# JuliaQuantumControl/QuantumPropagators.jl

Measured on AMD Instinct MI355X. Metric: Cheby prop_step!/s at N=2^20 CSR fp64 (2^20-row blocks advanced per second), higher is better.
Workload: dtype c128 (complex fp64); 1 GPU; BASELINE configs[1]: Cheby prop_step!, N=2^20 CSR sparse Hermitian H, 16 nnz/row, c128, int32 indices; N_total=1048576, rows_per_gpu=1048576, pattern=banded, n_coeffs=32, device_format=hrb (Hermitian-packed row blocks), parallelism=single GPU

## Files before the change

### quantumpropagators.jl_amd/csrc/device.h

```cpp
#pragma once

#include <hip/hip_runtime.h>

#include "layout_constants.h"

namespace qp {

#define QP_HIP(expr)                                                                         \
  do {                                                                                       \
    hipError_t e__ = (expr);                                                                 \
    if (e__ != hipSuccess) {                                                                 \
      (void)hipGetLastError();  \
      return qp::fail(QP_E_HIP, "%s failed: %s (%s:%d)", #expr, hipGetErrorString(e__), __FILE__, \
                      __LINE__);                                                             \
    }                                                                                        \
  } while (0)

constexpr int kRedBlocks = 256;
constexpr int kThreads = 256;

struct Stats;
struct Tuning;

struct DevMatrix {
  int format = QP_FMT_RBCSR;
  const Tuning* tun = nullptr;
  int64_t nrows = 0, ncols = 0, nnz = 0, stored = 0;
  int64_t nblocks = 0;
  int64_t* bptr = nullptr;
  int32_t* cols = nullptr;
  int64_t* cmeta = nullptr;
  int64_t colbytes = 0;
  double2* vals = nullptr;
  const double* vals_r = nullptr;
  int64_t* rowptr = nullptr;
  int lanes_per_row = 16;
  int64_t* lptr = nullptr;
  int32_t* lcols = nullptr;
  int64_t* lcmeta = nullptr;
  int64_t lcolbytes = 0;
  int32_t* lpos = nullptr;
  int64_t lstored = 0;
  const struct WalkPlan* walk = nullptr;
  const struct ColBlockPlan* cb = nullptr;
  const struct CodedVals* cv = nullptr;
  void* matfree = nullptr;
  int (*matfree_apply)(hipStream_t s, void* self, const double2* x, double2* y, double2 alpha, double2 beta,
                       Stats* st) = nullptr;
  double2* (*matfree_scratch)(void* self) = nullptr;
  int (*matfree_cheby)(hipStream_t s, void* self, const double2* x, const struct ChebyEpi& e, Stats* st) = nullptr;
};

constexpr int kWalkMaxNear = 8;
constexpr int kWalkHalo = 16;
struct WalkPlan {
  int valid = 0;
  int nn = 0, K = 0, z0 = 0;
  int S = 0;
  int xl = 0;
  int64_t glong = 0;
  int64_t glong1 = 0;
  int fd = 0;
  int64_t g = 0;
  int near[kWalkMaxNear] = {0};
  int64_t R0 = 0, R1 = 0, W0 = 0;
  int64_t U0 = 0;
  int ustride = 0;
  int32_t* edge_map = nullptr;
  int64_t n_edge = 0;
};

struct ColBlockPlan {
  int valid = 0;
  int log2w = 17;
  int P = 0;
  int rpt = 2;
  int max_seg = 0;
  int64_t ntiles = 0, nnz = 0;
  int32_t* segptr = nullptr;
  uint16_t* rowoff = nullptr;
  uint32_t* cols = nullptr;
  int64_t* map = nullptr;
  double2* vals = nullptr;
  double* vals_r = nullptr;
  int use_real = 0;
};
struct CodedVals {
// ... 6 lines not shown
  double* tab_r = nullptr;
  int use_real = 0;
};
constexpr int kCbMaxTilesPerWave = 8;
constexpr int kCbMaxSeg = 1024;

struct ChebyEpi {
  const double2* xloc;
  const double2* v0;
  double2* vout;
  const double2* acc_in;
  double2* acc_out;
  double2 c;
  double beta, a_prev, a;
  double2 phase;
  int apply_phase;
  double* check_partials;
  const int32_t* mirror = nullptr;
  double2* slab = nullptr;
  int acc_skip = 0;
  int n_defer = 0;
  double a_d1 = 0.0;
  double a_d2 = 0.0;
};

struct SyncArgs {
  unsigned* signal = nullptr;
  const unsigned* wait = nullptr;
  unsigned wait_target = 0;
  unsigned wait_from_wg = 0;
  unsigned* timeout_flag = nullptr;
  unsigned spin_limit = 1u << 28;
};

struct RowSet {
  const int32_t* block_map = nullptr;
  int64_t nmap = 0;
  bool count = true;
  SyncArgs sync;
  const struct WalkPlan* walk = nullptr;
  int reserve_cu = 0;
};

struct PlainEpi {
  double2* y;
  double2 alpha, beta;
  int beta_zero;
  const double2* norm_part = nullptr;
  const double2* xloc = nullptr;
  double2* qn_out = nullptr;
  double2* hess_slot = nullptr;
  double* norm_slot = nullptr;
  double dt = 1.0, norm_min = 0.0;
  unsigned* flag = nullptr;
  unsigned flag_value = 0;
};

struct Stats {
  uint64_t n_matvec = 0, n_cheby_steps = 0, n_newton_steps = 0, n_restarts = 0, n_launch = 0, n_graph_launch = 0;
  double spmv_bytes = 0;
};

int launch_spmv_cheby(hipStream_t s, const DevMatrix& A, const double2* x, const ChebyEpi& e, Stats* st,
                      const RowSet* rs = nullptr);
int launch_spmv_plain(hipStream_t s, const DevMatrix& A, const double2* x, const PlainEpi& e, Stats* st);
int launch_arnoldi_matvec_dots(hipStream_t s, const DevMatrix& A, const double2* x, const PlainEpi& e, const double2* Q,
                               int64_t ldq, int j, double2* partials, bool* launched, Stats* st);
bool arnoldi_onepass_fits(const DevMatrix& A, int m, int nvec);
int op_part_slots(int nvec);
int launch_arnoldi_onepass_sweep(hipStream_t s, const DevMatrix& A, const double2* start, double s0, double2* Q, int64_t ldq,
                                 double2* const a_buf[2], int m, int nvec, double2* const part[2], double2* gram, double2* hhat,
                                 double* svals, double* nu_dev, double dt, double2* hess_map, double* norms_map, double* nu_map,
                                 unsigned* flags_map, unsigned flag_value, Stats* st);
inline bool walk_shape_supported(int nn, int K, int z0, int xl = 0, int fd = 0) {
  if (fd) return fd == 1 && (xl == 0 || xl == 1) && K == 1 && nn >= 1 && nn <= 2 && (z0 == 0 || z0 == 1);
  if (xl) return (xl == 1 || xl == 2) && nn >= 1 && nn <= 2 && (K == 1 || K == 2) && (z0 == 0 || z0 == 1);
  return nn >= 1 && nn <= 4 && K >= 1 && K <= 4 && (z0 == 0 || z0 == 1);
}
inline bool walk2_shape_supported(int nn, int K, int z0) {
  return (z0 == 0 || z0 == 1) && nn >= 1 && nn <= 4 && K >= 1 && K <= 4;
}
int launch_hrb_walk2_cheby(hipStream_t s, const DevMatrix& A, const WalkPlan& P2, const double2* x, const ChebyEpi& e1,
                           const ChebyEpi& e2, const Tuning& tun, bool* launched);
int launch_hrb_walk_cheby(hipStream_t s, const DevMatrix& A, const double2* x, const ChebyEpi& e, const Tuning& tun,
                          bool* launched, const RowSet* rs = nullptr);
int launch_dense_gemv_cheby(hipStream_t s, const DevMatrix& A, const double2* x, const ChebyEpi& e, Stats* st);
int launch_dense_gemv_plain(hipStream_t s, const DevMatrix& A, const double2* x, const PlainEpi& e, Stats* st);
int launch_dense_zgemm_cheby(hipStream_t s, const DevMatrix& A, const double2* X, int batch, const ChebyEpi& e, Stats* st);
int launch_rbcsr_coded_cheby(hipStream_t s, const DevMatrix& A, const double2* x, const ChebyEpi& e, int64_t nblk,
                             const int32_t* bmap, const SyncArgs& sy, bool wide);
int launch_rbcsr_coded_plain(hipStream_t s, const DevMatrix& A, const double2* x, const PlainEpi& e, int64_t nblk,
                             const int32_t* bmap, const SyncArgs& sy);
int launch_colblock_cheby(hipStream_t s, const DevMatrix& A, const double2* x, const ChebyEpi& e, const Tuning& tun, bool* launched);
int launch_colblock_plain(hipStream_t s, const DevMatrix& A, const double2* x, const PlainEpi& e, const Tuning& tun, bool* launched);
int launch_colblock_gather(hipStream_t s, const ColBlockPlan& P, const double2* src, Stats* st);
int spmv_grid_size(const DevMatrix& A);
inline int dense_gemv_rows_per_wave(int64_t nrows) { return nrows >= 16384 ? 4 : 1; }
inline int dense_gemv_grid(int64_t nrows) {
  const int64_t per_wg = (int64_t)(kThreads / 64) * dense_gemv_rows_per_wave(nrows);
  return (int)((nrows + per_wg - 1) / per_wg);
}
constexpr int kDenseMinDensityPct = 75;
constexpr int kCbWavesPerCu = 16;
constexpr int kCbMinLog2N = 20;
constexpr int kWalkReserveCu = 8;
constexpr int kWalkEdgeSteps = 4;

struct Tuning {
  int rbcsr_variant = 15;
  int arnoldi_mode = 1;
  int arnoldi_onepass = 1;
  int sparse_controls = 1;
  int lattice_fill = 1;
  int arnoldi_fuse_dots = 1;
  int split_spin_log2 = 28;
  int split_dbg = 0;
  int split_mode = 2;
  int liouville_tile32_min_n = 260;
  int liouville_tile32_n = 2048;
  int liouville_fused_n = 320;
  int real_vals = 1;
  int block_map = 1;
  int stencil = 1;
  int acc_defer = 1;
  int cheby_graph = 0;
  int roctx = 0;
  int dense_auto = 1;
  int dense_panel_mfma = 1;
  int colblock = 1;
  int cb_log2w = 0;
  int small_nnz = 8192;
  int newton_pipeline = 1;
  int spmm_rows = 1;
  int spmm_rw = -1;
  int spmm_strip = 0;
  int hrb_walk = 1;
  int walk_waves = 0;
  int walk_pair = -1;
  int value_dict = 1;
  int walk_nt = -1;
  int walk_dbg = 0;
  int walk_min_blocks = 3072;
  int spmm_nt = 1;
};
int device_cu_count();
int* tuning_field(Tuning& t, const char* key);

constexpr int kCoefBlock = 32;
struct CoefBlock {
  double2 c[kCoefBlock];
};

int launch_real_part(hipStream_t s, double* out, const double2* v, int64_t n, Stats* st);
int launch_combine_planes(hipStream_t s, double2* vals, const double2* const* planes_dev, const double2* coefs,
                          int nplanes, int64_t n, double* vals_r, Stats* st);
int launch_sparse_planes_update(hipStream_t s, double2* vals, const double2* base, const int32_t* support, int64_t n_support,
                                const double2* support_vals, int nplanes, const double2* coefs, double* vals_r, Stats* st);


int launch_spmm_cheby(hipStream_t s, const int64_t* rowptr, const int32_t* cols, const double2* vals,
                      const double2* X, int64_t nrows, int64_t nnz, int b, const ChebyEpi& e, const Tuning& tun,
                      bool rows_kernel, const int32_t* order, Stats* st);
constexpr int kSpmmTileMaxEntries = 24;
constexpr int kSpmmTileSlots = 80;
struct SpmmTileShape {
  int nd = 0, K = 0, NN = 0;
  int dfar[kSpmmTileMaxEntries] = {0};
  int dnear[kSpmmTileMaxEntries] = {0};
};
constexpr int kSpmmTileTab = kSpmmTileSlots + 16 * kSpmmTileMaxEntries + 32;
struct SpmmTiles {
  bool built = false;
  int valid = 0;
  int knob = 0;
  SpmmTileShape shape;
  int64_t g = 0, sw = 0;
  int32_t* tiles = nullptr;
  int64_t ntiles = 0;
  int32_t* rest = nullptr;
  int64_t nrest = 0;
  int32_t* tab = nullptr;
  int T = 0;
};
int launch_spmm_tile_cheby(hipStream_t s, const int64_t* rowptr, const int32_t* cols, const double2* vals, const double2* X,
                           int64_t nrows, int64_t nnz, int b, const ChebyEpi& e, const Tuning& tun, const SpmmTiles& P, Stats* st);
inline bool spmm_uses_rows_kernel(const Tuning& tun, int b) { return tun.spmm_rows != 0 && b > 32; }
struct SmallObs {
  const int64_t* rowptr;
// ... 100 lines not shown
```

### quantumpropagators.jl_amd/csrc/engine_cheby.hip

```cpp
#include "engine.h"

void acc_schedule(const double* a, int n_coeffs, bool defer, qp_acc_defer* out) {
  const int nterms = n_coeffs - 1;
  std::vector<char> upd((size_t)nterms + 1, defer ? 0 : 1);
  if (defer) {
    int m0 = nterms;
    for (; m0 >= 1; m0 -= 3) upd[m0] = 1;
    if (m0 + 3 == 3) upd[1] = 1;
  }
  int last_upd = 0;
  for (int m = 1; m <= nterms; ++m) {
    qp_acc_defer& d = out[m - 1];
    d = qp_acc_defer{0, 0, 0.0, 0.0};
    if (upd[m]) {
      d.n_defer = m - last_upd - 1;
      d.a_d1 = (d.n_defer >= 1) ? a[m - 1] : 0.0;
      d.a_d2 = (d.n_defer == 2) ? a[m - 2] : 0.0;
      last_upd = m;
    } else {
      d.skip = 1;
    }
  }
}

// ... 13 lines not shown
}

extern "C" {

int qp_cheby_create(qp_ctx* ctx, int64_t n, qp_cheby** out) {
  QP_TRY
  if (!ctx || !out || n < 0) return qp::fail(QP_E_BAD_ARG, "qp_cheby_create: bad arguments");
  QP_CHECK(use(ctx));
  auto w = std::make_unique<qp_cheby>();
  w->ctx = ctx;
  w->n = n;
  QP_CHECK(dev_alloc(&w->bufA, (size_t)n));
  QP_CHECK(dev_alloc(&w->acc, (size_t)n));
  *out = w.release();
  return QP_OK;
  QP_CATCH
}

int qp_cheby_destroy(qp_cheby* w) {
  QP_TRY
  if (!w) return QP_OK;
  (void)hipSetDevice(w->ctx->device);
  (void)hipStreamSynchronize(w->ctx->stream);
  if (w->bufA) (void)hipFree(w->bufA);
  if (w->bufC) (void)hipFree(w->bufC);
  if (w->bufD) (void)hipFree(w->bufD);
  if (w->acc) (void)hipFree(w->acc);
  if (w->chk_part) (void)hipFree(w->chk_part);
  if (w->chk_out) (void)hipFree(w->chk_out);
  if (w->gexec) (void)hipGraphExecDestroy(w->gexec);
  delete w;
  return QP_OK;
  QP_CATCH
}

int qp_acc_schedule_host(const double* a, int n_coeffs, qp_acc_defer* out) {
  if (!a || !out || n_coeffs < 2) return qp::fail(QP_E_BAD_ARG, "qp_acc_schedule_host: bad arguments");
  acc_schedule(a, n_coeffs, true, out);
  return QP_OK;
}

int qp_cheby_term(qp_operator* op, const qp_state* x, int64_t xoff, const qp_state* v0, qp_state* vout,
                  const qp_state* acc_in, qp_state* acc_out, qp_c128 c, double beta, double a_prev, double a,
                  qp_c128 phase, const qp_acc_defer* defer) {
  QP_TRY
  const bool skip = defer && defer->skip;
  if (!op || !x || (!acc_out && !skip)) return qp::fail(QP_E_BAD_ARG, "qp_cheby_term: NULL argument");
  if (defer && !skip && (defer->n_defer < 0 || defer->n_defer > 2 || (defer->n_defer > 0 && !v0 && (defer->n_defer == 2 || !acc_in))))
    return qp::fail(QP_E_BAD_ARG, "qp_cheby_term: deferred accumulation needs v0");
  const int64_t nr = op->A.nrows;
  if (x->n != op->A.ncols || xoff < 0 || xoff + nr > x->n) return qp::fail(QP_E_BAD_ARG, "qp_cheby_term: x shape / offset mismatch");
  if ((v0 && v0->n != nr) || (vout && vout->n != nr) || (acc_in && acc_in->n != nr) || (acc_out && acc_out->n != nr))
    return qp::fail(QP_E_BAD_ARG, "qp_cheby_term: local vector length mismatch");
  auto overlaps = [&](const qp_state* s) { return s && s->d < x->d + x->n && x->d < s->d + s->n; };
  if (overlaps(vout) || overlaps(acc_out)) return qp::fail(QP_E_BAD_ARG, "qp_cheby_term: outputs must not overlap the gathered x");
  QP_CHECK(use(op->ctx));
  qp::ChebyEpi e;
  e.xloc = x->d + xoff;
  e.v0 = v0 ? v0->d : nullptr;
  e.vout = vout ? vout->d : nullptr;
  e.acc_in = (acc_in && !skip) ? acc_in->d : nullptr;
  e.acc_out = (acc_out && !skip) ? acc_out->d : nullptr;
  e.c = d2(c);
  e.beta = beta;
  e.a_prev = a_prev;
  e.a = a;
  e.phase = d2(phase);
  e.apply_phase = !(phase.re == 1.0 && phase.im == 0.0);
  e.check_partials = nullptr;
  set_defer(e, defer);
  return qp::launch_spmv_cheby(op->ctx->stream, op->A, x->d, e, &op->ctx->stats);
  QP_CATCH
}

static bool walk2_wanted(const qp_operator* op) {
  const qp::Tuning& tun = op->ctx->tun;
  const qp::WalkPlan& Q = op->walk2;
  const DevMatrix& A = op->A;
  if (!Q.valid || tun.walk_pair == 0 || !tun.hrb_walk || (tun.rbcsr_variant & 31) != 15 || A.walk != &op->walk || !op->walk.valid) return false;
  if (op->walk.R1 - op->walk.W0 < tun.walk_min_blocks) return false;
  if (tun.walk_pair == 1) return true;
  const double footprint = (double)(Q.z0 + Q.nn + Q.K) * kRB * (double)A.nblocks * (A.vals_r ? 8.0 : 16.0) + 64.0 * (double)A.nrows;
  if (footprint <= 230e6) return false;
  const int W = kRB - 2 * Q.near[Q.nn - 1];
  const int64_t S2 = (Q.g + W - 1) / W, Jz = ((Q.R1 - Q.W0) * (int64_t)kRB + Q.g - 1) / Q.g;
  const int64_t waves = tun.walk_waves > 0 ? tun.walk_waves : 4 * (int64_t)qp::device_cu_count();
  return Jz / std::max<int64_t>(1, waves / S2) >= 24;
}

int qp_operator_walk2_info(const qp_operator* op, int64_t out[8]) {
  QP_TRY
  if (!op || !out) return qp::fail(QP_E_BAD_ARG, "qp_operator_walk2_info: NULL argument");
  const bool on = walk2_wanted(op);
  const int W = on ? kRB - 2 * op->walk2.near[op->walk2.nn - 1] : 0;
  out[0] = on ? 1 : 0;
  out[1] = on ? op->walk2.W0 : 0;
  out[2] = on ? op->walk2.R1 : 0;
  out[3] = on ? op->walk2.n_edge : 0;
  out[4] = W;
  out[5] = on ? (op->walk2.g + W - 1) / W : 0;
  out[6] = out[7] = 0;
  if (on) {
    const qp::Tuning& tun = op->ctx->tun;
    const int64_t Jz = ((op->walk2.R1 - op->walk2.W0) * (int64_t)kRB + op->walk2.g - 1) / op->walk2.g;
    const int64_t waves = tun.walk_waves > 0 ? tun.walk_waves : 4 * (int64_t)qp::device_cu_count();
    const int64_t L = (Jz + std::max<int64_t>(1, waves / out[5]) - 1) / std::max<int64_t>(1, waves / out[5]);
    out[6] = L;
    out[7] = (Jz + L - 1) / L;
  }
  return QP_OK;
  QP_CATCH
}

static int cheby_step_launches(qp_cheby* w, qp_operator* op, qp_state* psi, const double* a, int n_coeffs, double beta,
                               cplx c, cplx phase, bool check_normalization) {
  qp_ctx* ctx = op->ctx;
  const DevMatrix& A = op->A;
  const int nterms = n_coeffs - 1;
  const int nwg = qp::spmv_grid_size(A);
  double2* P = psi->d;
  double2* B = w->bufA;
  double2* ACC = w->acc;
  double2* result = nullptr;
  std::vector<qp_acc_defer> sched((size_t)nterms);
  acc_schedule(a, n_coeffs, ctx->tun.acc_defer != 0, sched.data());
  bool pairs = !check_normalization && nterms >= 3 && w->bufC && w->bufD && walk2_wanted(op);
  double2 *cur = P, *prev = nullptr;
  double2* spare[2] = {w->bufC, w->bufD};
  bool updated = false;
  auto fill = [&](qp::ChebyEpi& e, int m, const double2* x) {
    e.a_prev = updated ? 0.0 : a[0];
    set_defer(e, &sched[m - 1]);
    if (sched[m - 1].skip) {
      e.acc_in = nullptr;
      e.acc_out = nullptr;
    } else {
      updated = true;
    }
    e.xloc = x;
    e.c = d2(c);
    e.beta = beta;
    e.a = a[m];
    e.phase = d2(phase);
    e.apply_phase = (m == nterms) ? 1 : 0;
  };
  for (int m = 1; m <= nterms; ++m) {
    const bool last = (m == nterms);
    qp::ChebyEpi e;
    if (m == 1) {
      e.v0 = nullptr;
      e.vout = last ? nullptr : B;
      e.acc_in = nullptr;
      e.acc_out = ACC;
      result = ACC;
    } else if (pairs && m + 1 <= nterms && !(sched[m - 1].skip == 0 && sched[m].skip == 0)) {
      const bool last2 = (m + 1 == nterms);
      const bool updated_before = updated;
      qp::ChebyEpi e1, e2;
      e1.v0 = prev;
      e1.vout = spare[0];
      e1.acc_in = updated ? ACC : nullptr;
      e1.acc_out = ACC;
      e1.check_partials = nullptr;
      fill(e1, m, cur);
      e2.v0 = cur;
      e2.vout = last2 ? nullptr : spare[1];
      e2.acc_in = updated ? ACC : nullptr;
      e2.acc_out = ACC;
      e2.check_partials = nullptr;
      fill(e2, m + 1, spare[0]);
      bool launched = false;
      {
        const qp::ScopedRange mv_range(ctx->tun.roctx != 0 || qp::ranges_enabled_by_env(), "matrix-vector product");
        QP_CHECK(qp::launch_hrb_walk2_cheby(ctx->stream, A, op->walk2, cur, e1, e2, ctx->tun, &launched));
        if (launched) {
          qp::RowSet rs;
          rs.block_map = op->walk2.edge_map;
          rs.nmap = op->walk2.n_edge;
          rs.count = false;
          QP_CHECK(qp::launch_spmv_cheby(ctx->stream, A, spare[0], e2, &ctx->stats, &rs));
          ctx->stats.n_launch++;
          ctx->stats.n_matvec += 2;
          ctx->stats.spmv_bytes += 2.0 * (20.0 * (double)A.nnz + 4.0 * (double)(A.nrows + 1) + 80.0 * (double)A.nrows);
        }
      }
      if (launched) {
        result = ACC;
        double2* const y = spare[0];
        double2* const z = spare[1];
        spare[0] = cur;
        spare[1] = prev;
        prev = y;
        cur = z;
        ++m;
        continue;
      }
      updated = updated_before;
      pairs = false;
    }
    if (m > 1) {
      e.v0 = prev;
      e.vout = last ? nullptr : prev;
      e.acc_in = updated ? ACC : nullptr;
      e.acc_out = (last && cur != P && !pairs) ? P : ACC;
      result = e.acc_out;
    }
    fill(e, m, cur);
    e.check_partials = (check_normalization && m >= 2) ? w->chk_part : nullptr;
    {
      const qp::ScopedRange mv_range(ctx->tun.roctx != 0 || qp::ranges_enabled_by_env(), "matrix-vector product");
      QP_CHECK(qp::launch_spmv_cheby(ctx->stream, A, cur, e, &ctx->stats));
    }
    if (e.check_partials)
      QP_CHECK(qp::launch_reduce_triples(ctx->stream, w->chk_part, nwg, w->chk_out + 3 * (m - 1), &ctx->stats));
    if (m == 1) {
      c *= 2.0;
      prev = P;
      cur = B;
    } else {
      std::swap(cur, prev);
    }
  }
  if (result != P)
    QP_HIP(hipMemcpyAsync(P, result, (size_t)psi->n * sizeof(double2), hipMemcpyDeviceToDevice, ctx->stream));
  return QP_OK;
}

int qp_cheby_step(qp_cheby* w, qp_operator* op, qp_state* psi, const double* a, int n_coeffs, double Delta,
                  double E_min, double dt, double wrk_dt, double limit, int check_normalization) {
  QP_TRY
  if (!w || !op || !psi || !a) return qp::fail(QP_E_BAD_ARG, "qp_cheby_step: NULL argument");
  if (op->A.nrows != op->A.ncols || psi->n != op->A.nrows || w->n != psi->n)
    return qp::fail(QP_E_BAD_ARG, "qp_cheby_step: shape mismatch");
  {
    const double x = std::fabs(dt), y = std::fabs(wrk_dt);
    if (!(std::fabs(x - y) <= 1.4901161193847656e-08 * std::max(x, y)))
      return qp::fail(QP_E_DT_MISMATCH, "wrk was initialized for dt=%g, not dt=abs(%g)", wrk_dt, dt);
  }
  if (n_coeffs < 2) return qp::fail(QP_E_TOO_FEW_COEFFS, "Need at least 2 Chebychev coefficients");
  if (!(Delta > 0)) return qp::fail(QP_E_BAD_ARG, "Delta must be positive");
  qp_ctx* ctx = op->ctx;
  QP_CHECK(use(ctx));
  const qp::ScopedRange step_range(ctx->tun.roctx != 0 || qp::ranges_enabled_by_env(), "prop_step!");
  const double beta = (Delta / 2) + E_min;
  cplx c = (dt > 0) ? cplx(0, -2.0) / Delta : cplx(0, 2.0) / Delta;
  const cplx phase = std::exp(cplx(0, -1) * beta * dt);
  const int nterms = n_coeffs - 1;
  const DevMatrix& A = op->A;
  const int nwg = qp::spmv_grid_size(A);
  if (check_normalization) {
    if (w->chk_wg < nwg) {
      if (w->chk_part) QP_HIP(hipFree(w->chk_part));
      QP_CHECK(dev_alloc(&w->chk_part, (size_t)3 * nwg));
      w->chk_wg = nwg;
    }
    if (w->chk_terms < nterms) {
      if (w->chk_out) QP_HIP(hipFree(w->chk_out));
      QP_CHECK(dev_alloc(&w->chk_out, (size_t)3 * nterms));
      w->chk_terms = nterms;
    }
  }
  if (nterms >= 3 && !check_normalization && !w->bufC && walk2_wanted(op)) {
    QP_CHECK(dev_alloc(&w->bufC, (size_t)w->n));
    QP_CHECK(dev_alloc(&w->bufD, (size_t)w->n));
  }
  bool done = false;
  if (ctx->tun.cheby_graph && !check_normalization && ctx->stream != nullptr && ctx->stream != hipStreamLegacy) {
    qp_cheby::GraphKey key;
    key.vals = A.vals_r ? (const void*)A.vals_r : (const void*)A.vals;
    key.cols = A.cols;
// ... 566 lines not shown
```

### quantumpropagators.jl_amd/csrc/kernels_walk2.hip

```cpp
#include "kernels_walk2_impl.h"

namespace qp {

QP_WALK2_DEFINE(walk2_launch_nn4, 4)

int launch_hrb_walk2_cheby(hipStream_t s, const DevMatrix& A, const WalkPlan& P2, const double2* x, const ChebyEpi& e1,
                           const ChebyEpi& e2, const Tuning& tun, bool* launched) {
  *launched = false;
  if (!P2.valid || A.format != QP_FMT_HRB || !walk2_shape_supported(P2.nn, P2.K, P2.z0) || P2.xl || P2.fd || P2.g % kRB) return QP_OK;
  if (!e1.v0 || e1.check_partials || e2.check_partials || e1.mirror || e2.mirror || e1.xloc != x) return QP_OK;
  Walk2Geom G;
  const int dmax = P2.near[P2.nn - 1];
  G.W = kRB - 2 * dmax;
  if (G.W < 16) return QP_OK;
  G.S2 = (int)((P2.g + G.W - 1) / G.W);
  const int64_t Jz = ((P2.R1 - P2.W0) * (int64_t)kRB + P2.g - 1) / P2.g;
  const int64_t waves = tun.walk_waves > 0 ? tun.walk_waves : (int64_t)kWalk2Waves * device_cu_count();
  const int64_t nseg_target = std::max<int64_t>(1, waves / G.S2);
  G.L = (int)((Jz + nseg_target - 1) / nseg_target);
  G.nseg = (int)((Jz + G.L - 1) / G.L);
  const int64_t ntask = std::max<int64_t>((int64_t)G.nseg * G.S2, 1);
  G.n_walk_wg = (int)((ntask + kWalk2Waves - 1) / kWalk2Waves);
  G.ntask = G.n_walk_wg * kWalk2Waves;
  G.xlast = A.ncols - 1;
  G.vend = (P2.R1 + (int64_t)P2.K * P2.S) * (int64_t)kRB;
  HrbArrays H{A.bptr, A.cmeta, reinterpret_cast<const char*>(A.cols), A.lptr, A.lcmeta,
              reinterpret_cast<const char*>(A.lcols), reinterpret_cast<const int4*>(A.lpos)};
  ChebyOp op1{e1}, op2{e2};
  const double value_bytes = (double)(P2.z0 + P2.nn + P2.K) * kRB * (double)A.nblocks * (A.vals_r ? 8.0 : 16.0);
  const int ntm = tun.walk_nt >= 0 ? tun.walk_nt : (value_bytes <= 300e6 ? 1 : 0);
  bool ok = false;
  switch (P2.nn) {
#define QP_WALK2_CASE(NN_)                                                                                   \
  case NN_:                                                                                                  \
    ok = A.vals_r ? walk2_launch_nn##NN_##_f64(s, A.vals_r, x, P2, G, H, A.nrows, op1, op2, ntm)                \
                  : walk2_launch_nn##NN_##_c128(s, A.vals, x, P2, G, H, A.nrows, op1, op2, ntm);                \
    break;
    QP_WALK2_CASE(1)
    QP_WALK2_CASE(2)
    QP_WALK2_CASE(3)
    QP_WALK2_CASE(4)
#undef QP_WALK2_CASE
    default: break;
  }
  if (!ok) return QP_OK;
  QP_HIP(hipGetLastError());
  *launched = true;
  return QP_OK;
}

}
```

### quantumpropagators.jl_amd/csrc/kernels_walk2_impl.h

```cpp
#pragma once
#include <atomic>

#include "kernels_walk_impl.h"

namespace qp {

constexpr int kWalk2Waves = 4;

template <int NN, int K>
struct Walk2Lds {
  static constexpr int XW = kRB + 2 * kWalkHalo, AW = kRB + kWalkHalo;
  static constexpr int kWin = XW + NN * AW;
  static constexpr int kFifo = K * K + K * (K + 1) / 2;
  static constexpr int kPerWave = kWin + kRB * kFifo;
  static constexpr size_t kBytesPerWave = sizeof(double2) * (size_t)kPerWave;
};

struct Walk2Geom {
  int L = 0, nseg = 0, ntask = 0, n_walk_wg = 0;
  int S2 = 0;
  int W = 0;
  int64_t xlast = 0;
  int64_t vend = 0;
};

template <int NU>
struct Walk2Step {
  double2 ua[NU];
  double2 xnew;
  double2 p, acc1;
  double2 acc2;
  double2 hx, ha;
};

template <class VT, int NN, int K, int Z0, int NTM>
__global__ __launch_bounds__(64 * kWalk2Waves) void hrb_walk2_kernel(const VT* __restrict__ uvals, const double2* __restrict__ x,
                                                                      WalkPlan P, Walk2Geom G, HrbArrays H, int64_t nrows,
                                                                      ChebyOp op1, ChebyOp op2) {
  constexpr int NL = NN + K;
  constexpr int NU = Z0 + NN + K;
  constexpr int NH = Z0 + NN;
  using Lds = Walk2Lds<NN, K>;
  constexpr int XW = Lds::XW, AW = Lds::AW;
  static_assert(NN <= 4, "the near value halos share one register: sixteen lanes each");
  extern __shared__ double2 walk2_lds[];
  const int wave = __builtin_amdgcn_readfirstlane(threadIdx.x >> 6);
  const int lane = threadIdx.x & 63;
  const unsigned wg = xcd_remap(blockIdx.x, G.n_walk_wg);
  const int task = (int)wg * kWalk2Waves + wave;
  for (int64_t idx = task; idx < P.n_edge; idx += G.ntask)
    hrb_edge_block<VT>(H, uvals, x, (int64_t)__builtin_amdgcn_readfirstlane(P.edge_map[idx]), lane, nrows, op1);
  const int seg = task / G.S2, col = task - seg * G.S2;
  if (seg >= G.nseg) return;
  const int64_t g = P.g;
  const int64_t zb = P.W0 * (int64_t)kRB, ze = P.R1 * (int64_t)kRB;
  const int Jz = (int)((ze - zb + g - 1) / g);
  const int j0 = seg * G.L, j1 = min(j0 + G.L, Jz);
  if (j0 >= j1) return;
  const int dmax = P.near[NN - 1];
  const int64_t coff = (int64_t)col * G.W - dmax;
  const bool owner = lane >= dmax && lane < kRB - dmax && coff + lane < g;
  double2* __restrict__ xwin = walk2_lds + (size_t)wave * Lds::kPerWave;
  double2* __restrict__ fifo = xwin + Lds::kWin;
  const int64_t rlo = P.R0 * (int64_t)kRB, vmax = G.vend - 1, rmax = G.xlast, nlast = nrows - 1;
  auto vpos = [&](int64_t r) __attribute__((always_inline)) -> int64_t {
    return P.U0 + ((r >> 6) - P.R0) * (int64_t)P.ustride + (r & 63);
  };
  auto clampv = [&](int64_t r) __attribute__((always_inline)) -> int64_t { return min(max(r, rlo), vmax); };
  ChebyOp opl1{op1.e}, opl2{op2.e};
  opl1.e.mirror = opl2.e.mirror = nullptr;
  opl1.e.check_partials = opl2.e.check_partials = nullptr;
  const double2* __restrict__ pp = op1.e.v0;
  const double2* __restrict__ acc1p = op1.e.acc_in;
  const double2* __restrict__ acc2p = op2.e.acc_in;
  const int hq = lane >> 4, ht = lane & 15;
  const int hd = P.near[hq < NN ? hq : NN - 1];
  const int hoff_x = (hq & 1) ? kRB + min(ht, dmax - 1) : -dmax + min(ht, dmax - 1);
  const int hslot = Z0 + (hq < NN ? hq : NN - 1);
  auto row_of = [&](int t) __attribute__((always_inline)) -> int64_t { return zb + (int64_t)t * g + coff; };
  auto load_step = [&](int t, Walk2Step<NU>& w) __attribute__((always_inline)) {
    const int64_t r0 = row_of(t);
    const int64_t r = clampv(r0 + lane);
    const VT* __restrict__ v = uvals + vpos(r);
#pragma unroll
    for (int u = 0; u < NU; ++u) w.ua[u] = ld_val<(NTM & 1) != 0>(v + (size_t)u * 64);
    w.xnew = x[min(max(r0 + lane + K * g, (int64_t)0), rmax)];
    const int64_t rc = min(max(r0 + lane, (int64_t)0), nlast);
    w.p = pp[rc];
    w.acc1 = acc1p ? acc1p[rc] : x[lane];
    w.acc2 = acc2p ? acc2p[min(max(r0 + lane - K * g, (int64_t)0), nlast)] : x[lane];
    w.hx = x[min(max(r0 + hoff_x, (int64_t)0), rmax)];
    w.ha = ld_val<false>(uvals + vpos(clampv(r0 - hd + min(ht, hd - 1))) + (size_t)hslot * 64);
  };
  const bool hx_on = hq < 2 && ht < dmax;
  const int hx_pos = hx_on ? ((hq & 1) ? kWalkHalo + kRB + ht : kWalkHalo - dmax + ht) : kWalkHalo + lane;
  const bool ha_on = hq < NN && ht < hd;
  const int ha_pos = XW + (hq < NN ? hq : 0) * AW + (ha_on ? kWalkHalo - hd + ht : kWalkHalo + lane);

  const int t0 = j0 - K;
  const int nsteps = (j1 - j0) + 2 * K;
  double2 xr[2 * K + 1], yr[2 * K + 1];
  {
    const int64_t r0 = row_of(t0);
#pragma unroll
    for (int m = -K; m < K; ++m) xr[K + m] = x[min(max(r0 + lane + m * g, (int64_t)0), rmax)];
  }
#pragma unroll
  for (int i = 0; i <= 2 * K; ++i) yr[i] = make_double2(0.0, 0.0);
  double2 nh[K + 1][NH];
#pragma unroll
  for (int a = 0; a <= K; ++a)
#pragma unroll
    for (int u = 0; u < NH; ++u) nh[a][u] = make_double2(0.0, 0.0);
  auto foff = [](int m) __attribute__((always_inline)) -> int { return (m - 1) * K + (m - 1) * m / 2; };
#pragma unroll
  for (int m = 1; m <= K; ++m)
#pragma unroll
    for (int a = 1; a <= m; ++a)
      fifo[(foff(m) + (K + m - a)) * kRB + lane] =
          ld_val<false>(uvals + vpos(clampv(row_of(t0) + lane - (int64_t)a * g)) + (size_t)(Z0 + NN + (m - 1)) * 64);
  int hp[K];
#pragma unroll
  for (int m = 1; m <= K; ++m) hp[m - 1] = 0;
  auto fpos = [&](int m, int age) __attribute__((always_inline)) -> int {
    const int q = hp[m - 1] - age;
    return foff(m) + (q < 0 ? q + K + m : q);
  };

  Walk2Step<NU> wa, wb;
  load_step(t0, wa);
  int tau = 0;
  auto step = [&](const Walk2Step<NU>& cu, Walk2Step<NU>& nx, auto has_next) __attribute__((always_inline)) {
    const int t = t0 + tau;
    xr[2 * K] = cu.xnew;
    if constexpr (decltype(has_next)::value) load_step(t + 1, nx);
#pragma unroll
    for (int u = 0; u < NH; ++u) nh[K][u] = cu.ua[u];
    xwin[kWalkHalo + lane] = xr[K];
    xwin[hx_pos] = sel2(hx_on, cu.hx, xr[K]);
#pragma unroll
// ... 69 lines not shown
#pragma unroll
    for (int i = 0; i < NN; ++i) xwin[XW + i * AW + kWalkHalo + lane] = nh[0][Z0 + i];
    __builtin_amdgcn_fence(__ATOMIC_RELEASE, "wavefront");
    __builtin_amdgcn_wave_barrier();
    __builtin_amdgcn_fence(__ATOMIC_ACQUIRE, "wavefront");
    {
      double2 za[NN], zyl[NN], zyu[NN];
#pragma unroll
      for (int i = 0; i < NN; ++i) {
        const int d = P.near[i];
        za[i] = xwin[XW + i * AW + kWalkHalo + lane - d];
        zyl[i] = xwin[kWalkHalo + lane - d];
        zyu[i] = xwin[kWalkHalo + lane + d];
      }
      double2 s0 = make_double2(0.0, 0.0), s1 = make_double2(0.0, 0.0);
#pragma unroll
      for (int l = 0; l < NL; ++l) {
        double2 a, xv;
        if (l < K) {
          const int m = K - l;
          a = fzl[m - 1];
          xv = yr[K - m];
        } else {
          const int i = NN - 1 - (l - K);
          a = za[i];
          xv = zyl[i];
        }
        if (l & 1) cfma_conj(s1, a, xv);
        else cfma_conj(s0, a, xv);
      }
#pragma unroll
      for (int u = 0; u < NU; ++u) {
        double2 a, xv;
        if (u < Z0) {
          a = nh[0][u];
          xv = yr[K];
        } else if (u < Z0 + NN) {
          a = nh[0][u];
          xv = zyu[u - Z0];
        } else {
          const int m = u - Z0 - NN + 1;
          a = fzu[m - 1];
          xv = yr[K + m];
        }
        if (u & 1) cfma(s1, a, xv);
        else cfma(s0, a, xv);
      }
      ChebyOp::Pre pre;
      pre.xi = yr[K];
      pre.v0 = xr[0];
      pre.acc = acc2p ? cu.acc2 : make_double2(0.0, 0.0);
      const double2 zv = opl2.term(make_double2(s0.x + s1.x, s0.y + s1.y), pre);
      const int c = t - K;
      const int64_t row = row_of(c) + lane;
      if (owner && c >= j0 && c < j1 && row < ze) opl2.finish(row, zv, pre);
    }
    __builtin_amdgcn_fence(__ATOMIC_RELEASE, "wavefront");
    __builtin_amdgcn_wave_barrier();
    __builtin_amdgcn_fence(__ATOMIC_ACQUIRE, "wavefront");
#pragma unroll
    for (int i = 0; i < 2 * K; ++i) {
      xr[i] = xr[i + 1];
      yr[i] = yr[i + 1];
    }
#pragma unroll
    for (int a = 0; a < K; ++a)
#pragma unroll
      for (int u = 0; u < NH; ++u) nh[a][u] = nh[a + 1][u];
    ++tau;
  };
  int n = nsteps;
  for (; n > 2; n -= 2) {
    step(wa, wb, std::true_type());
    step(wb, wa, std::true_type());
  }
  if (n == 2) {
    step(wa, wb, std::true_type());
    step(wb, wa, std::false_type());
  } else {
    step(wa, wb, std::false_type());
  }
}

template <class VT, int NN, int K, int Z0, int NTM>
static bool launch2_instance(hipStream_t s, const VT* uvals, const double2* x, const WalkPlan& P, const Walk2Geom& G,
                             const HrbArrays& H, int64_t nrows, const ChebyOp& op1, const ChebyOp& op2) {
  constexpr size_t lds = Walk2Lds<NN, K>::kBytesPerWave * kWalk2Waves;
  static_assert(lds <= 160 * 1024, "four wavefronts' windows and FIFOs fit the compute unit's LDS");
  auto kern = &hrb_walk2_kernel<VT, NN, K, Z0, NTM>;
  static std::atomic<unsigned char> opted[64];
  int dev = 0;
  if (hipGetDevice(&dev) != hipSuccess || dev < 0 || dev >= 64) return false;
  unsigned char st = opted[dev].load(std::memory_order_acquire);
  if (st == 0) {
    st = hipFuncSetAttribute(reinterpret_cast<const void*>(kern), hipFuncAttributeMaxDynamicSharedMemorySize, (int)lds) == hipSuccess ? 1 : 2;
    if (st == 2) (void)hipGetLastError();
    opted[dev].store(st, std::memory_order_release);
  }
  if (st != 1) return false;
  hipLaunchKernelGGL(kern, dim3((unsigned)G.n_walk_wg), dim3(64 * kWalk2Waves), lds, s, uvals, x, P, G, H, nrows, op1, op2);
  return true;
}

template <class VT, int NN>
static bool launch2_shape(hipStream_t s, const VT* uvals, const double2* x, const WalkPlan& P, const Walk2Geom& G,
                          const HrbArrays& H, int64_t nrows, const ChebyOp& op1, const ChebyOp& op2, int ntm) {
  if (P.nn != NN) return false;
#define QP_WALK2(K_, Z0_)                                                                              \
  return (ntm & 1) ? launch2_instance<VT, NN, K_, Z0_, 1>(s, uvals, x, P, G, H, nrows, op1, op2)         \
                   : launch2_instance<VT, NN, K_, Z0_, 0>(s, uvals, x, P, G, H, nrows, op1, op2);
  switch (P.K * 10 + P.z0) {
    case 10: QP_WALK2(1, 0)
    case 11: QP_WALK2(1, 1)
    case 20: QP_WALK2(2, 0)
    case 21: QP_WALK2(2, 1)
    case 30: QP_WALK2(3, 0)
    case 31: QP_WALK2(3, 1)
    case 40: QP_WALK2(4, 0)
    case 41: QP_WALK2(4, 1)
    default: return false;
  }
#undef QP_WALK2
}

#define QP_WALK2_DECL(NAME)                                                                                                   \
  bool NAME##_c128(hipStream_t s, const double2* uvals, const double2* x, const WalkPlan& P, const Walk2Geom& G, const HrbArrays& H, \
                   int64_t nrows, const ChebyOp& op1, const ChebyOp& op2, int ntm);                                                  \
  bool NAME##_f64(hipStream_t s, const double* uvals, const double2* x, const WalkPlan& P, const Walk2Geom& G, const HrbArrays& H,    \
                  int64_t nrows, const ChebyOp& op1, const ChebyOp& op2, int ntm);
QP_WALK2_DECL(walk2_launch_nn1)
QP_WALK2_DECL(walk2_launch_nn2)
QP_WALK2_DECL(walk2_launch_nn3)
QP_WALK2_DECL(walk2_launch_nn4)
#undef QP_WALK2_DECL
#define QP_WALK2_DEFINE(NAME, NN_)                                                                                            \
  bool NAME##_c128(hipStream_t s, const double2* uvals, const double2* x, const WalkPlan& P, const Walk2Geom& G, const HrbArrays& H, \
                   int64_t nrows, const ChebyOp& op1, const ChebyOp& op2, int ntm) {                                                 \
    return launch2_shape<double2, NN_>(s, uvals, x, P, G, H, nrows, op1, op2, ntm);                                                  \
  }                                                                                                                                   \
  bool NAME##_f64(hipStream_t s, const double* uvals, const double2* x, const WalkPlan& P, const Walk2Geom& G, const HrbArrays& H,    \
                  int64_t nrows, const ChebyOp& op1, const ChebyOp& op2, int ntm) {                                                   \
    return launch2_shape<double, NN_>(s, uvals, x, P, G, H, nrows, op1, op2, ntm);                                                    \
  }

}
```

### quantumpropagators.jl_amd/csrc/operator_layout.h

```cpp
#pragma once

#include <algorithm>
#include <chrono>
#include <cstdlib>
#include <cstring>
#include <system_error>
#include <thread>

#include "layout_constants.h"

namespace qp {
template <class T>
struct NoInitAlloc {
  using value_type = T;
  NoInitAlloc() = default;
  template <class U>
  NoInitAlloc(const NoInitAlloc<U>&) {}
  T* allocate(size_t n) { return static_cast<T*>(::operator new(n * sizeof(T))); }
  void deallocate(T* p, size_t) { ::operator delete(p); }
  template <class U, class... A>
  void construct(U* p, A&&... a) {
    if constexpr (sizeof...(A) > 0) ::new ((void*)p) U(std::forward<A>(a)...);
  }
  template <class U>
  bool operator==(const NoInitAlloc<U>&) const { return true; }
  template <class U>
  bool operator!=(const NoInitAlloc<U>&) const { return false; }
};
template <class T>
using HostVec = std::vector<T, NoInitAlloc<T>>;
}
using qp::cplx;
using qp::kRB;

inline unsigned host_threads() {
  static const unsigned n = [] {
    unsigned hw = std::max(1u, std::thread::hardware_concurrency());
    if (FILE* f = std::fopen("/sys/fs/cgroup/cpu.max", "r")) {
      char q[32] = {0};
      long period = 0;
      if (std::fscanf(f, "%31s %ld", q, &period) == 2 && std::strcmp(q, "max") != 0 && period > 0) {
        const long quota = std::atol(q) / period;
        if (quota >= 1) hw = std::min<unsigned>(hw, (unsigned)quota);
      }
      std::fclose(f);
    }
    unsigned cap = 16;
    if (const char* e = std::getenv("QP_HOST_THREADS")) {
      const long v = std::atol(e);
      if (v >= 1) cap = (unsigned)std::min<long>(v, 256);
    }
    return std::max(1u, std::min(cap, hw > 2 ? hw - 1 : hw));
  }();
  return n;
}

struct BuildTrace {
  std::chrono::steady_clock::time_point t = std::chrono::steady_clock::now();
  const bool on = std::getenv("QP_BUILD_TRACE") != nullptr;
  void mark(const char* what) {
    if (!on) return;
    const auto now = std::chrono::steady_clock::now();
    std::fprintf(stderr, "[qp build] %-44s %9.2f ms\n", what, std::chrono::duration<double, std::milli>(now - t).count());
    t = now;
  }
};

template <class F>
inline void parallel_rows(int64_t n, F&& fn, int64_t serial_below = (int64_t)1 << 16) {
  const unsigned hw = host_threads();
  if (n < serial_below || hw == 1) {
    fn((int64_t)0, n);
    return;
  }
  std::vector<std::thread> th;
  const int64_t chunk = (n + hw - 1) / hw;
  int64_t done = 0;
  try {
    for (unsigned t = 0; t < hw; ++t) {
      const int64_t a = (int64_t)t * chunk, b = std::min(n, a + chunk);
      if (a >= b) break;
      th.emplace_back([&fn, a, b] { fn(a, b); });
      done = b;
    }
  } catch (const std::system_error&) {
  }
  for (auto& x : th) x.join();
  if (done < n) fn(done, n);
}

template <class T>
inline void parallel_copy(T* dst, const T* src, size_t n) {
// ... 131 lines not shown
```

Before: 1043 prop_step/s.

## Rebalance two-term walk segments around edge work and add dedicated edge kernel

Moves the walk2 segment geometry into a shared cut helper that shortens the first segments by a fixed number of steps, so waves that also handle edge blocks get less walk work. It adds a policy that picks fewer, fixed-count waves when the operator's value footprint fits a resident-size threshold, and spreads edge tasks across workgroups by wave-major indexing. The second-term edge pass now uses a lightweight one-wave-per-block kernel in place of the generic row-set SpMV. On the last term the result can be accumulated directly into psi, skipping a copy. The uneven segment split adds indexing complexity and depends on the edge-step heuristic.

```diff
diff --git a/quantumpropagators.jl_amd/csrc/device.h b/quantumpropagators.jl_amd/csrc/device.h
--- a/quantumpropagators.jl_amd/csrc/device.h
+++ b/quantumpropagators.jl_amd/csrc/device.h
@@ -3,6 +3,7 @@
 #include <hip/hip_runtime.h>
 
 #include "layout_constants.h"
+#include "walk2_cut.h"
 
 namespace qp {
 
@@ -175,6 +176,16 @@
 }
 int launch_hrb_walk2_cheby(hipStream_t s, const DevMatrix& A, const WalkPlan& P2, const double2* x, const ChebyEpi& e1,
                            const ChebyEpi& e2, const Tuning& tun, bool* launched);
+int launch_hrb_walk2_edges(hipStream_t s, const DevMatrix& A, const WalkPlan& P2, const double2* y, const ChebyEpi& e2);
+struct Walk2Policy {
+  bool resident = false;
+  int64_t waves = 0;
+  int ntm = 0;
+  int edge_steps = 0;
+  int spread = 1;
+};
+Walk2Policy walk2_policy(const DevMatrix& A, const WalkPlan& P2, const Tuning& tun);
+Walk2Cut walk2_cut_of(const DevMatrix& A, const WalkPlan& P2, const Tuning& tun);
 int launch_hrb_walk_cheby(hipStream_t s, const DevMatrix& A, const double2* x, const ChebyEpi& e, const Tuning& tun,
                           bool* launched, const RowSet* rs = nullptr);
 int launch_dense_gemv_cheby(hipStream_t s, const DevMatrix& A, const double2* x, const ChebyEpi& e, Stats* st);
@@ -197,6 +208,9 @@
 constexpr int kCbWavesPerCu = 16;
 constexpr int kCbMinLog2N = 20;
 constexpr int kWalkReserveCu = 8;
+constexpr int kWalk2EdgeSteps = 4;
+constexpr int kWalk2ResidentWaves = 1024;
+constexpr double kWalk2ResidentBytes = 256e6;
 constexpr int kWalkEdgeSteps = 4;
 
 struct Tuning {
diff --git a/quantumpropagators.jl_amd/csrc/engine_cheby.hip b/quantumpropagators.jl_amd/csrc/engine_cheby.hip
--- a/quantumpropagators.jl_amd/csrc/engine_cheby.hip
+++ b/quantumpropagators.jl_amd/csrc/engine_cheby.hip
@@ -119,10 +119,11 @@
   if (tun.walk_pair == 1) return true;
   const double footprint = (double)(Q.z0 + Q.nn + Q.K) * kRB * (double)A.nblocks * (A.vals_r ? 8.0 : 16.0) + 64.0 * (double)A.nrows;
   if (footprint <= 230e6) return false;
+  const qp::Walk2Policy pol = qp::walk2_policy(A, Q, tun);
   const int W = kRB - 2 * Q.near[Q.nn - 1];
+  if (W < 16) return false;
   const int64_t S2 = (Q.g + W - 1) / W, Jz = ((Q.R1 - Q.W0) * (int64_t)kRB + Q.g - 1) / Q.g;
-  const int64_t waves = tun.walk_waves > 0 ? tun.walk_waves : 4 * (int64_t)qp::device_cu_count();
-  return Jz / std::max<int64_t>(1, waves / S2) >= 24;
+  return Jz / std::max<int64_t>(1, pol.waves / S2) >= 24;
 }
 
 int qp_operator_walk2_info(const qp_operator* op, int64_t out[8]) {
@@ -138,12 +139,9 @@
   out[5] = on ? (op->walk2.g + W - 1) / W : 0;
   out[6] = out[7] = 0;
   if (on) {
-    const qp::Tuning& tun = op->ctx->tun;
-    const int64_t Jz = ((op->walk2.R1 - op->walk2.W0) * (int64_t)kRB + op->walk2.g - 1) / op->walk2.g;
-    const int64_t waves = tun.walk_waves > 0 ? tun.walk_waves : 4 * (int64_t)qp::device_cu_count();
-    const int64_t L = (Jz + std::max<int64_t>(1, waves / out[5]) - 1) / std::max<int64_t>(1, waves / out[5]);
-    out[6] = L;
-    out[7] = (Jz + L - 1) / L;
+    const qp::Walk2Cut cut = qp::walk2_cut_of(op->A, op->walk2, op->ctx->tun);
+    out[6] = cut.longest();
+    out[7] = cut.nseg;
   }
   return QP_OK;
   QP_CATCH
@@ -206,23 +204,30 @@
       e2.acc_out = ACC;
       e2.check_partials = nullptr;
       fill(e2, m + 1, spare[0]);
+      const bool to_psi = last2 && e2.acc_out && spare[1] == P;
+      if (to_psi) e2.acc_out = P;
       bool launched = false;
       {
         const qp::ScopedRange mv_range(ctx->tun.roctx != 0 || qp::ranges_enabled_by_env(), "matrix-vector product");
         QP_CHECK(qp::launch_hrb_walk2_cheby(ctx->stream, A, op->walk2, cur, e1, e2, ctx->tun, &launched));
         if (launched) {
-          qp::RowSet rs;
-          rs.block_map = op->walk2.edge_map;
-          rs.nmap = op->walk2.n_edge;
-          rs.count = false;
-          QP_CHECK(qp::launch_spmv_cheby(ctx->stream, A, spare[0], e2, &ctx->stats, &rs));
+          if (ctx->tun.walk_dbg & 512) {
+            qp::RowSet rs;
+            rs.block_map = op->walk2.edge_map;
+            rs.nmap = op->walk2.n_edge;
+            rs.count = false;
+            QP_CHECK(qp::launch_spmv_cheby(ctx->stream, A, spare[0], e2, &ctx->stats, &rs));
+          } else {
+            QP_CHECK(qp::launch_hrb_walk2_edges(ctx->stream, A, op->walk2, spare[0], e2));
+            ctx->stats.n_launch++;
+          }
           ctx->stats.n_launch++;
           ctx->stats.n_matvec += 2;
           ctx->stats.spmv_bytes += 2.0 * (20.0 * (double)A.nnz + 4.0 * (double)(A.nrows + 1) + 80.0 * (double)A.nrows);
         }
       }
       if (launched) {
-        result = ACC;
+        result = to_psi ? P : ACC;
         double2* const y = spare[0];
         double2* const z = spare[1];
         spare[0] = cur;
diff --git a/quantumpropagators.jl_amd/csrc/kernels_walk2.hip b/quantumpropagators.jl_amd/csrc/kernels_walk2.hip
--- a/quantumpropagators.jl_amd/csrc/kernels_walk2.hip
+++ b/quantumpropagators.jl_amd/csrc/kernels_walk2.hip
@@ -4,31 +4,46 @@
 
 QP_WALK2_DEFINE(walk2_launch_nn4, 4)
 
+Walk2Policy walk2_policy(const DevMatrix& A, const WalkPlan& P2, const Tuning& tun) {
+  Walk2Policy p;
+  const double value_bytes = (double)(P2.z0 + P2.nn + P2.K) * kRB * (double)A.nblocks * (A.vals_r ? 8.0 : 16.0);
+  p.resident = value_bytes + 5.0 * 16.0 * (double)A.nrows <= kWalk2ResidentBytes;
+  p.waves = tun.walk_waves > 0 ? tun.walk_waves : (p.resident ? kWalk2ResidentWaves : kWalk2Waves * device_cu_count());
+  p.ntm = tun.walk_nt >= 0 ? tun.walk_nt : (p.resident ? 0 : (value_bytes <= 300e6 ? 1 : 0));
+  const int dbg_steps = (tun.walk_dbg >> 4) & 15;
+  p.edge_steps = dbg_steps ? dbg_steps - 1 : kWalk2EdgeSteps;
+  p.spread = (tun.walk_dbg & 256) ? 0 : 1;
+  return p;
+}
+Walk2Cut walk2_cut_of(const DevMatrix& A, const WalkPlan& P2, const Tuning& tun) {
+  const Walk2Policy p = walk2_policy(A, P2, tun);
+  return walk2_cut(P2.g, P2.near[P2.nn - 1], P2.R1 - P2.W0, P2.n_edge, p.waves, p.edge_steps);
+}
+
 int launch_hrb_walk2_cheby(hipStream_t s, const DevMatrix& A, const WalkPlan& P2, const double2* x, const ChebyEpi& e1,
                            const ChebyEpi& e2, const Tuning& tun, bool* launched) {
   *launched = false;
   if (!P2.valid || A.format != QP_FMT_HRB || !walk2_shape_supported(P2.nn, P2.K, P2.z0) || P2.xl || P2.fd || P2.g % kRB) return QP_OK;
   if (!e1.v0 || e1.check_partials || e2.check_partials || e1.mirror || e2.mirror || e1.xloc != x) return QP_OK;
+  const Walk2Policy pol = walk2_policy(A, P2, tun);
+  const Walk2Cut cut = walk2_cut_of(A, P2, tun);
+  if (cut.W < 16 || cut.nseg < 1) return QP_OK;
   Walk2Geom G;
-  const int dmax = P2.near[P2.nn - 1];
-  G.W = kRB - 2 * dmax;
-  if (G.W < 16) return QP_OK;
-  G.S2 = (int)((P2.g + G.W - 1) / G.W);
-  const int64_t Jz = ((P2.R1 - P2.W0) * (int64_t)kRB + P2.g - 1) / P2.g;
-  const int64_t waves = tun.walk_waves > 0 ? tun.walk_waves : (int64_t)kWalk2Waves * device_cu_count();
-  const int64_t nseg_target = std::max<int64_t>(1, waves / G.S2);
-  G.L = (int)((Jz + nseg_target - 1) / nseg_target);
-  G.nseg = (int)((Jz + G.L - 1) / G.L);
-  const int64_t ntask = std::max<int64_t>((int64_t)G.nseg * G.S2, 1);
-  G.n_walk_wg = (int)((ntask + kWalk2Waves - 1) / kWalk2Waves);
-  G.ntask = G.n_walk_wg * kWalk2Waves;
+  G.W = cut.W;
+  G.S2 = cut.S2;
+  G.L = cut.L;
+  G.nseg = cut.nseg;
+  G.edge_segs = cut.edge_segs;
+  G.edge_steps = cut.edge_steps;
+  G.spread = pol.spread;
+  G.n_walk_wg = cut.n_wg;
+  G.ntask = (int)cut.tasks;
   G.xlast = A.ncols - 1;
   G.vend = (P2.R1 + (int64_t)P2.K * P2.S) * (int64_t)kRB;
   HrbArrays H{A.bptr, A.cmeta, reinterpret_cast<const char*>(A.cols), A.lptr, A.lcmeta,
               reinterpret_cast<const char*>(A.lcols), reinterpret_cast<const int4*>(A.lpos)};
   ChebyOp op1{e1}, op2{e2};
-  const double value_bytes = (double)(P2.z0 + P2.nn + P2.K) * kRB * (double)A.nblocks * (A.vals_r ? 8.0 : 16.0);
-  const int ntm = tun.walk_nt >= 0 ? tun.walk_nt : (value_bytes <= 300e6 ? 1 : 0);
+  const int ntm = pol.ntm;
   bool ok = false;
   switch (P2.nn) {
 #define QP_WALK2_CASE(NN_)                                                                                   \
@@ -49,4 +64,18 @@
   return QP_OK;
 }
 
+int launch_hrb_walk2_edges(hipStream_t s, const DevMatrix& A, const WalkPlan& P2, const double2* y, const ChebyEpi& e2) {
+  if (P2.n_edge <= 0) return QP_OK;
+  if (e2.check_partials || e2.mirror) return fail(QP_E_INTERNAL, "two-term walk: the edge launch has no check / mirror epilogue");
+  HrbArrays H{A.bptr, A.cmeta, reinterpret_cast<const char*>(A.cols), A.lptr, A.lcmeta,
+              reinterpret_cast<const char*>(A.lcols), reinterpret_cast<const int4*>(A.lpos)};
+  ChebyOp op{e2};
+  if (A.vals_r)
+    hipLaunchKernelGGL(hrb_walk2_edge_kernel<double>, dim3((unsigned)P2.n_edge), dim3(64), 0, s, A.vals_r, y, P2.edge_map, P2.n_edge, H, A.nrows, op);
+  else
+    hipLaunchKernelGGL(hrb_walk2_edge_kernel<double2>, dim3((unsigned)P2.n_edge), dim3(64), 0, s, A.vals, y, P2.edge_map, P2.n_edge, H, A.nrows, op);
+  QP_HIP(hipGetLastError());
+  return QP_OK;
 }
+
+}
diff --git a/quantumpropagators.jl_amd/csrc/kernels_walk2_impl.h b/quantumpropagators.jl_amd/csrc/kernels_walk2_impl.h
--- a/quantumpropagators.jl_amd/csrc/kernels_walk2_impl.h
+++ b/quantumpropagators.jl_amd/csrc/kernels_walk2_impl.h
@@ -18,6 +18,8 @@
 
 struct Walk2Geom {
   int L = 0, nseg = 0, ntask = 0, n_walk_wg = 0;
+  int edge_segs = 0, edge_steps = 0;
+  int spread = 0;
   int S2 = 0;
   int W = 0;
   int64_t xlast = 0;
@@ -47,7 +49,7 @@
   const int wave = __builtin_amdgcn_readfirstlane(threadIdx.x >> 6);
   const int lane = threadIdx.x & 63;
   const unsigned wg = xcd_remap(blockIdx.x, G.n_walk_wg);
-  const int task = (int)wg * kWalk2Waves + wave;
+  const int task = G.spread ? wave * G.n_walk_wg + (int)wg : (int)wg * kWalk2Waves + wave;
   for (int64_t idx = task; idx < P.n_edge; idx += G.ntask)
     hrb_edge_block<VT>(H, uvals, x, (int64_t)__builtin_amdgcn_readfirstlane(P.edge_map[idx]), lane, nrows, op1);
   const int seg = task / G.S2, col = task - seg * G.S2;
@@ -55,7 +57,8 @@
   const int64_t g = P.g;
   const int64_t zb = P.W0 * (int64_t)kRB, ze = P.R1 * (int64_t)kRB;
   const int Jz = (int)((ze - zb + g - 1) / g);
-  const int j0 = seg * G.L, j1 = min(j0 + G.L, Jz);
+  const int j0 = seg * G.L - min(seg, G.edge_segs) * G.edge_steps;
+  const int j1 = min((seg + 1) * G.L - min(seg + 1, G.edge_segs) * G.edge_steps, Jz);
   if (j0 >= j1) return;
   const int dmax = P.near[NN - 1];
   const int64_t coff = (int64_t)col * G.W - dmax;
@@ -291,6 +294,15 @@
   }
 }
 
+template <class VT>
+__global__ __launch_bounds__(64) void hrb_walk2_edge_kernel(const VT* __restrict__ uvals, const double2* __restrict__ x,
+                                                            const int32_t* __restrict__ edge_map, int64_t n_edge, HrbArrays H,
+                                                            int64_t nrows, ChebyOp op) {
+  const int64_t idx = blockIdx.x;
+  if (idx >= n_edge) return;
+  hrb_edge_block<VT>(H, uvals, x, (int64_t)__builtin_amdgcn_readfirstlane(edge_map[idx]), (int)threadIdx.x, nrows, op);
+}
+
 template <class VT, int NN, int K, int Z0, int NTM>
 static bool launch2_instance(hipStream_t s, const VT* uvals, const double2* x, const WalkPlan& P, const Walk2Geom& G,
                              const HrbArrays& H, int64_t nrows, const ChebyOp& op1, const ChebyOp& op2) {
diff --git a/quantumpropagators.jl_amd/csrc/operator_layout.h b/quantumpropagators.jl_amd/csrc/operator_layout.h
--- a/quantumpropagators.jl_amd/csrc/operator_layout.h
+++ b/quantumpropagators.jl_amd/csrc/operator_layout.h
@@ -8,6 +8,7 @@
 #include <thread>
 
 #include "layout_constants.h"
+#include "walk2_cut.h"
 
 namespace qp {
 template <class T>
diff --git a/quantumpropagators.jl_amd/csrc/walk2_cut.h b/quantumpropagators.jl_amd/csrc/walk2_cut.h
--- /dev/null
+++ b/quantumpropagators.jl_amd/csrc/walk2_cut.h
@@ -0,0 +1,50 @@
+#pragma once
+
+#include <algorithm>
+#include <cstdint>
+
+#include "layout_constants.h"
+
+namespace qp {
+struct Walk2Cut {
+  int W = 0;
+  int S2 = 0;
+  int64_t Jz = 0;
+  int L = 0;
+  int nseg = 0;
+  int edge_segs = 0;
+  int edge_steps = 0;
+  int n_wg = 0;
+  int64_t tasks = 0;
+  int64_t edge_tasks = 0;
+  int64_t seg_begin(int64_t seg) const { return seg * L - std::min<int64_t>(seg, edge_segs) * edge_steps; }
+  int64_t seg_end(int64_t seg) const { return std::min(seg_begin(seg + 1), Jz); }
+  int64_t longest() const {
+    int64_t m = 0;
+    for (int64_t s = 0; s < nseg; ++s) m = std::max(m, seg_end(s) - seg_begin(s));
+    return m;
+  }
+};
+inline Walk2Cut walk2_cut(int64_t g, int dmax, int64_t region_blocks, int64_t n_edge, int64_t waves, int edge_steps) {
+  Walk2Cut c;
+  c.W = (int)kRB - 2 * dmax;
+  if (c.W < 1 || g < 1 || region_blocks < 1) return c;
+  c.S2 = (int)((g + c.W - 1) / c.W);
+  c.Jz = (region_blocks * (int64_t)kRB + g - 1) / g;
+  const int64_t nseg_target = std::max<int64_t>(1, std::max<int64_t>(waves, 1) / c.S2);
+  c.edge_steps = std::max(edge_steps, 0);
+  int64_t esegs = c.edge_steps > 0 ? std::min(nseg_target, (std::max<int64_t>(n_edge, 0) + c.S2 - 1) / c.S2) : 0;
+  const int64_t total = c.Jz + esegs * c.edge_steps;
+  const int64_t L = std::max<int64_t>(c.edge_steps + 1, (total + nseg_target - 1) / nseg_target);
+  int64_t nseg = (total + L - 1) / L;
+  while (nseg * L - std::min(esegs, nseg) * c.edge_steps < c.Jz) ++nseg;
+  while (nseg > 1 && (nseg - 1) * L - std::min(esegs, nseg - 1) * c.edge_steps >= c.Jz) --nseg;
+  c.L = (int)L;
+  c.nseg = (int)nseg;
+  c.edge_segs = (int)std::min(esegs, nseg);
+  c.n_wg = (int)((nseg * c.S2 + 3) / 4);
+  c.tasks = (int64_t)c.n_wg * 4;
+  c.edge_tasks = std::min<int64_t>(std::max<int64_t>(n_edge, 0), c.tasks);
+  return c;
+}
+}
```

After: 1044 prop_step/s, median of 5. Within noise of the previous version (+0.0%).
